# PaddlePaddle/PaddleNLP

Hardware: NVIDIA H100
Metric: tokens/sec Llama-3.2-3B seq4096 bf16 pretrain step (global, all GPUs) (higher is better)
Workload: dtype bf16

## Files before the change

paddlenlp_b200/csrc/common.cuh:

```cuda
#pragma once
#include <cuda.h>
#include <cuda_bf16.h>
#include <cuda_runtime.h>
#include <stdint.h>
#include <stdio.h>

namespace b200 {

typedef __nv_bfloat16 bf16;

__device__ __forceinline__ uint32_t smem_u32(const void* p) {
  return static_cast<uint32_t>(__cvta_generic_to_shared(p));
}
__device__ __forceinline__ void named_bar_sync(uint32_t id, uint32_t nthreads) {
  asm volatile("bar.sync %0, %1;" ::"r"(id), "r"(nthreads) : "memory");
}

__device__ __forceinline__ void pdl_wait() { asm volatile("griddepcontrol.wait;" ::: "memory"); }
__device__ __forceinline__ void pdl_launch_dependents() { asm volatile("griddepcontrol.launch_dependents;" ::: "memory"); }

__device__ __forceinline__ void mbar_init(uint64_t* bar, uint32_t count) {
  asm volatile("mbarrier.init.shared::cta.b64 [%0], %1;" ::"r"(smem_u32(bar)), "r"(count) : "memory");
}
__device__ __forceinline__ void fence_mbar_init() {
  asm volatile("fence.mbarrier_init.release.cluster;" ::: "memory");
}
__device__ __forceinline__ void fence_proxy_async_smem() {
  asm volatile("fence.proxy.async.shared::cta;" ::: "memory");
}
__device__ __forceinline__ void mbar_arrive_expect_tx(uint64_t* bar, uint32_t bytes) {
  asm volatile("mbarrier.arrive.expect_tx.shared::cta.b64 _, [%0], %1;" ::"r"(smem_u32(bar)), "r"(bytes)
               : "memory");
}
__device__ __forceinline__ void mbar_arrive(uint64_t* bar) {
  asm volatile("mbarrier.arrive.shared::cta.b64 _, [%0];" ::"r"(smem_u32(bar)) : "memory");
}
__device__ __forceinline__ bool mbar_try_wait(uint64_t* bar, uint32_t parity) {
  uint32_t ok;
  asm volatile(
      "{\n\t.reg .pred P;\n\t"
      "mbarrier.try_wait.parity.shared::cta.b64 P, [%1], %2;\n\t"
      "selp.u32 %0, 1, 0, P;\n\t}\n"
      : "=r"(ok)
      : "r"(smem_u32(bar)), "r"(parity)
      : "memory");
  return ok != 0;
}
__device__ __forceinline__ void mbar_wait(uint64_t* bar, uint32_t parity) {
  if (mbar_try_wait(bar, parity)) return;
  long long t0 = clock64();
  uint32_t spins = 0;
  while (!mbar_try_wait(bar, parity)) {
    if ((++spins & 0x3FFu) == 0 && (clock64() - t0) > 8000000000LL) {
      printf("[b200 watchdog] mbarrier wait timed out: block %d thread %d bar 0x%x parity %u\n", (int)blockIdx.x,
             (int)threadIdx.x, smem_u32(bar), parity);
      __trap();
    }
  }
}
__device__ __forceinline__ void mbar_wait_nocall(uint64_t* bar, uint32_t parity) {
  if (mbar_try_wait(bar, parity)) return;
  long long t0 = clock64();
  uint32_t spins = 0;
  while (!mbar_try_wait(bar, parity)) {
    if ((++spins & 0x3FFu) == 0 && (clock64() - t0) > 8000000000LL) __trap();
  }
}

__device__ __forceinline__ void tma_prefetch_desc(const CUtensorMap* tm) {
  asm volatile("prefetch.tensormap [%0];" ::"l"(reinterpret_cast<uint64_t>(tm)) : "memory");
}
__device__ __forceinline__ void tma_load_2d(const CUtensorMap* tm, uint64_t* bar, void* smem_dst, int c0, int c1) {
  asm volatile(
      "cp.async.bulk.tensor.2d.shared::cluster.global.mbarrier::complete_tx::bytes [%0], [%1, {%3, %4}], [%2];"
      ::"r"(smem_u32(smem_dst)), "l"(reinterpret_cast<uint64_t>(tm)), "r"(smem_u32(bar)), "r"(c0), "r"(c1)
      : "memory");
}
__device__ __forceinline__ void bulk_load(void* smem_dst, const void* src, uint32_t bytes, uint64_t* bar) {
  asm volatile("cp.async.bulk.shared::cluster.global.mbarrier::complete_tx::bytes [%0], [%1], %2, [%3];" ::"r"(smem_u32(smem_dst)),
               "l"(src), "r"(bytes), "r"(smem_u32(bar))
               : "memory");
}
__device__ __forceinline__ void tma_load_4d(const CUtensorMap* tm, uint64_t* bar, void* smem_dst, int c0, int c1,
                                            int c2, int c3) {
  asm volatile(
      "cp.async.bulk.tensor.4d.shared::cluster.global.mbarrier::complete_tx::bytes [%0], [%1, {%3, %4, %5, %6}], [%2];"
      ::"r"(smem_u32(smem_dst)), "l"(reinterpret_cast<uint64_t>(tm)), "r"(smem_u32(bar)), "r"(c0), "r"(c1), "r"(c2),
      "r"(c3)
      : "memory");
}
__device__ __forceinline__ void tma_reduce_add_4d(const CUtensorMap* tm, const void* smem_src, int c0, int c1, int c2,
                                                  int c3) {
  asm volatile("cp.reduce.async.bulk.tensor.4d.global.shared::cta.add.tile.bulk_group [%0, {%2, %3, %4, %5}], [%1];" ::"l"(
                   reinterpret_cast<uint64_t>(tm)),
               "r"(smem_u32(smem_src)), "r"(c0), "r"(c1), "r"(c2), "r"(c3)
               : "memory");
}
__device__ __forceinline__ void tma_reduce_add_2d(const CUtensorMap* tm, uint32_t smem_src, int c0, int c1) {
  asm volatile("cp.reduce.async.bulk.tensor.2d.global.shared::cta.add.tile.bulk_group [%0, {%2, %3}], [%1];" ::"l"(
                   reinterpret_cast<uint64_t>(tm)),
               "r"(smem_src), "r"(c0), "r"(c1)
               : "memory");
}
__device__ __forceinline__ void tma_store_2d(const CUtensorMap* tm, uint32_t smem_src, int c0, int c1) {
  asm volatile("cp.async.bulk.tensor.2d.global.shared::cta.bulk_group [%0, {%2, %3}], [%1];" ::"l"(reinterpret_cast<uint64_t>(tm)),
               "r"(smem_src), "r"(c0), "r"(c1)
               : "memory");
}
__device__ __forceinline__ void tma_prefetch_l2_2d(const CUtensorMap* tm, int c0, int c1) {
  asm volatile("cp.async.bulk.prefetch.tensor.2d.L2.global.tile [%0, {%1, %2}];" ::"l"(reinterpret_cast<uint64_t>(tm)), "r"(c0),
               "r"(c1)
               : "memory");
}
__device__ __forceinline__ void tma_store_commit() { asm volatile("cp.async.bulk.commit_group;" ::: "memory"); }
template <int N>
__device__ __forceinline__ void tma_store_wait_read() {
  asm volatile("cp.async.bulk.wait_group.read %0;" ::"n"(N) : "memory");
}
template <int N>
__device__ __forceinline__ void tma_store_wait() {
  asm volatile("cp.async.bulk.wait_group %0;" ::"n"(N) : "memory");
}

__device__ __forceinline__ uint64_t wgmma_desc_sw128(uint32_t saddr, uint32_t lbo_bytes, uint32_t sbo_bytes) {
  uint64_t d = 0;
  d |= static_cast<uint64_t>((saddr & 0x3FFFFu) >> 4);
  d |= static_cast<uint64_t>((lbo_bytes >> 4) & 0x3FFFu) << 16;
  d |= static_cast<uint64_t>((sbo_bytes >> 4) & 0x3FFFu) << 32;
  d |= static_cast<uint64_t>(1) << 62;
  return d;
}
__device__ __forceinline__ void wgmma_fence() { asm volatile("wgmma.fence.sync.aligned;" ::: "memory"); }
__device__ __forceinline__ void wgmma_commit() { asm volatile("wgmma.commit_group.sync.aligned;" ::: "memory"); }
template <int N>
__device__ __forceinline__ void wgmma_wait() { asm volatile("wgmma.wait_group.sync.aligned %0;" ::"n"(N) : "memory"); }
template <int R>
__device__ __forceinline__ void setmaxnreg_dec() { asm volatile("setmaxnreg.dec.sync.aligned.u32 %0;" ::"n"(R)); }
template <int R>
__device__ __forceinline__ void setmaxnreg_inc() { asm volatile("setmaxnreg.inc.sync.aligned.u32 %0;" ::"n"(R)); }

template <int TA, int TB>
__device__ __forceinline__ void wgmma_m64n256k16(float (&d)[128], uint64_t desc_a, uint64_t desc_b, uint32_t accumulate) {
  asm volatile(
      "{\n\t.reg .pred p;\n\tsetp.ne.b32 p, %130, 0;\n\t"
      "wgmma.mma_async.sync.aligned.m64n256k16.f32.bf16.bf16 "
      "{%0, %1, %2, %3, %4, %5, %6, %7, %8, %9, %10, %11, %12, %13, %14, %15, %16, %17, %18, %19, %20, %21, %22, %23, %24, %25, %26, %27, %28, %29, %30, %31, %32, %33, %34, %35, %36, %37, %38, %39, %40, %41, %42, %43, %44, %45, %46, %47, %48, %49, %50, %51, %52, %53, %54, %55, %56, %57, %58, %59, %60, %61, %62, %63, %64, %65, %66, %67, %68, %69, %70, %71, %72, %73, %74, %75, %76, %77, %78, %79, %80, %81, %82, %83, %84, %85, %86, %87, %88, %89, %90, %91, %92, %93, %94, %95, %96, %97, %98, %99, %100, %101, %102, %103, %104, %105, %106, %107, %108, %109, %110, %111, %112, %113, %114, %115, %116, %117, %118, %119, %120, %121, %122, %123, %124, %125, %126, %127}, %128, %129, p, 1, 1, %131, %132;\n\t}\n"
      : "+f"(d[0]), "+f"(d[1]), "+f"(d[2]), "+f"(d[3]), "+f"(d[4]), "+f"(d[5]), "+f"(d[6]), "+f"(d[7]), "+f"(d[8]), "+f"(d[9]), "+f"(d[10]), "+f"(d[11]), "+f"(d[12]), "+f"(d[13]), "+f"(d[14]), "+f"(d[15]), "+f"(d[16]), "+f"(d[17]), "+f"(d[18]), "+f"(d[19]), "+f"(d[20]), "+f"(d[21]), "+f"(d[22]), "+f"(d[23]), "+f"(d[24]), "+f"(d[25]), "+f"(d[26]), "+f"(d[27]), "+f"(d[28]), "+f"(d[29]), "+f"(d[30]), "+f"(d[31]), "+f"(d[32]), "+f"(d[33]), "+f"(d[34]), "+f"(d[35]), "+f"(d[36]), "+f"(d[37]), "+f"(d[38]), "+f"(d[39]), "+f"(d[40]), "+f"(d[41]), "+f"(d[42]), "+f"(d[43]), "+f"(d[44]), "+f"(d[45]), "+f"(d[46]), "+f"(d[47]), "+f"(d[48]), "+f"(d[49]), "+f"(d[50]), "+f"(d[51]), "+f"(d[52]), "+f"(d[53]), "+f"(d[54]), "+f"(d[55]), "+f"(d[56]), "+f"(d[57]), "+f"(d[58]), "+f"(d[59]), "+f"(d[60]), "+f"(d[61]), "+f"(d[62]), "+f"(d[63]), "+f"(d[64]), "+f"(d[65]), "+f"(d[66]), "+f"(d[67]), "+f"(d[68]), "+f"(d[69]), "+f"(d[70]), "+f"(d[71]), "+f"(d[72]), "+f"(d[73]), "+f"(d[74]), "+f"(d[75]), "+f"(d[76]), "+f"(d[77]), "+f"(d[78]), "+f"(d[79]), "+f"(d[80]), "+f"(d[81]), "+f"(d[82]), "+f"(d[83]), "+f"(d[84]), "+f"(d[85]), "+f"(d[86]), "+f"(d[87]), "+f"(d[88]), "+f"(d[89]), "+f"(d[90]), "+f"(d[91]), "+f"(d[92]), "+f"(d[93]), "+f"(d[94]), "+f"(d[95]), "+f"(d[96]), "+f"(d[97]), "+f"(d[98]), "+f"(d[99]), "+f"(d[100]), "+f"(d[101]), "+f"(d[102]), "+f"(d[103]), "+f"(d[104]), "+f"(d[105]), "+f"(d[106]), "+f"(d[107]), "+f"(d[108]), "+f"(d[109]), "+f"(d[110]), "+f"(d[111]), "+f"(d[112]), "+f"(d[113]), "+f"(d[114]), "+f"(d[115]), "+f"(d[116]), "+f"(d[117]), "+f"(d[118]), "+f"(d[119]), "+f"(d[120]), "+f"(d[121]), "+f"(d[122]), "+f"(d[123]), "+f"(d[124]), "+f"(d[125]), "+f"(d[126]), "+f"(d[127])
      : "l"(desc_a), "l"(desc_b), "r"(accumulate), "n"(TA), "n"(TB));
}
template <int TA, int TB>
__device__ __forceinline__ void wgmma_m64n64k16(float (&d)[32], uint64_t desc_a, uint64_t desc_b, uint32_t accumulate) {
  asm volatile(
      "{\n\t.reg .pred p;\n\tsetp.ne.b32 p, %34, 0;\n\t"
      "wgmma.mma_async.sync.aligned.m64n64k16.f32.bf16.bf16 "
      "{%0, %1, %2, %3, %4, %5, %6, %7, %8, %9, %10, %11, %12, %13, %14, %15, %16, %17, %18, %19, %20, %21, %22, %23, %24, %25, %26, %27, %28, %29, %30, %31}, %32, %33, p, 1, 1, %35, %36;\n\t}\n"
      : "+f"(d[0]), "+f"(d[1]), "+f"(d[2]), "+f"(d[3]), "+f"(d[4]), "+f"(d[5]), "+f"(d[6]), "+f"(d[7]), "+f"(d[8]), "+f"(d[9]), "+f"(d[10]), "+f"(d[11]), "+f"(d[12]), "+f"(d[13]), "+f"(d[14]), "+f"(d[15]), "+f"(d[16]), "+f"(d[17]), "+f"(d[18]), "+f"(d[19]), "+f"(d[20]), "+f"(d[21]), "+f"(d[22]), "+f"(d[23]), "+f"(d[24]), "+f"(d[25]), "+f"(d[26]), "+f"(d[27]), "+f"(d[28]), "+f"(d[29]), "+f"(d[30]), "+f"(d[31])
      : "l"(desc_a), "l"(desc_b), "r"(accumulate), "n"(TA), "n"(TB));
}
template <int TA, int TB>
__device__ __forceinline__ void wgmma_m64n128k16(float (&d)[64], uint64_t desc_a, uint64_t desc_b, uint32_t accumulate) {
  asm volatile(
      "{\n\t.reg .pred p;\n\tsetp.ne.b32 p, %66, 0;\n\t"
      "wgmma.mma_async.sync.aligned.m64n128k16.f32.bf16.bf16 "
      "{%0, %1, %2, %3, %4, %5, %6, %7, %8, %9, %10, %11, %12, %13, %14, %15, %16, %17, %18, %19, %20, %21, %22, %23, %24, %25, %26, %27, %28, %29, %30, %31, %32, %33, %34, %35, %36, %37, %38, %39, %40, %41, %42, %43, %44, %45, %46, %47, %48, %49, %50, %51, %52, %53, %54, %55, %56, %57, %58, %59, %60, %61, %62, %63}, %64, %65, p, 1, 1, %67, %68;\n\t}\n"
      : "+f"(d[0]), "+f"(d[1]), "+f"(d[2]), "+f"(d[3]), "+f"(d[4]), "+f"(d[5]), "+f"(d[6]), "+f"(d[7]), "+f"(d[8]), "+f"(d[9]), "+f"(d[10]), "+f"(d[11]), "+f"(d[12]), "+f"(d[13]), "+f"(d[14]), "+f"(d[15]), "+f"(d[16]), "+f"(d[17]), "+f"(d[18]), "+f"(d[19]), "+f"(d[20]), "+f"(d[21]), "+f"(d[22]), "+f"(d[23]), "+f"(d[24]), "+f"(d[25]), "+f"(d[26]), "+f"(d[27]), "+f"(d[28]), "+f"(d[29]), "+f"(d[30]), "+f"(d[31]), "+f"(d[32]), "+f"(d[33]), "+f"(d[34]), "+f"(d[35]), "+f"(d[36]), "+f"(d[37]), "+f"(d[38]), "+f"(d[39]), "+f"(d[40]), "+f"(d[41]), "+f"(d[42]), "+f"(d[43]), "+f"(d[44]), "+f"(d[45]), "+f"(d[46]), "+f"(d[47]), "+f"(d[48]), "+f"(d[49]), "+f"(d[50]), "+f"(d[51]), "+f"(d[52]), "+f"(d[53]), "+f"(d[54]), "+f"(d[55]), "+f"(d[56]), "+f"(d[57]), "+f"(d[58]), "+f"(d[59]), "+f"(d[60]), "+f"(d[61]), "+f"(d[62]), "+f"(d[63])
      : "l"(desc_a), "l"(desc_b), "r"(accumulate), "n"(TA), "n"(TB));
}
template <int TB>
// ... 152 lines not shown
```

paddlenlp_b200/csrc/fa_bwd.cu:

```cuda
#include <climits>

#include "../../include/b200nlp.h"
#include "common.cuh"
#include "host_util.h"

namespace b200 {
namespace fab {

constexpr int BKV = 64;
constexpr int NUM_THREADS = 256;

struct Params {
  const bf16 *q, *k, *v, *dout;
  int64_t ldq, ldk, ldv, lddo;
  int S, B, nh, kvh, Spad;
  float scale, scale_log2;
  const float* lse2;
  const float* delta;
  const int* mask_start;
  float* dq_acc;
  float* dk_acc;
  float* dv_acc;
};

// ... 74 lines not shown
          ldsm_x4(sV + swz<D>(kr, kc * 2 + ((lane >> 3) & 1)), bv);
          mma_bf16_16816(s[2 * np], a, b[0], b[1]);
          mma_bf16_16816(s[2 * np + 1], a, b[2], b[3]);
          mma_bf16_16816(dp[2 * np], ad, bv[0], bv[1]);
          mma_bf16_16816(dp[2 * np + 1], ad, bv[2], bv[3]);
        }
      }
#pragma unroll
      for (int h = 0; h < 2; ++h) {
        const int rl = rg * 16 + g + 8 * h, r = q0 + rl;
        const float lse2 = s_lse[rl], dl = s_delta[rl];
#pragma unroll
        for (int nt = 0; nt < NT; ++nt) {
          float pv[2], dsv[2];
#pragma unroll
          for (int e = 0; e < 2; ++e) {
            const int c = kv0 + cs * NT * 8 + nt * 8 + 2 * tq + e;
            bool dead = c > r;
            if constexpr (MASK) {
              if (!dead && c < p.S) dead = r >= __ldg(p.mask_start + tok0 + c);
            }
            pv[e] = dead ? 0.f : fast_exp2(fmaf(s[nt][2 * h + e], p.scale_log2, -lse2));
            dsv[e] = pv[e] * (dp[nt][2 * h + e] - dl) * p.scale;
          }
          const int cc = cs * NT + nt;
          asm volatile("st.shared.b32 [%0], %1;" ::"r"(sP + swz64(rl, cc) + tq * 4), "r"(pack_bf16x2(pv[0], pv[1])) : "memory");
          asm volatile("st.shared.b32 [%0], %1;" ::"r"(sdS + swz64(rl, cc) + tq * 4), "r"(pack_bf16x2(dsv[0], dsv[1])) : "memory");
        }
      }
    }
    __syncthreads();

#pragma unroll
    for (int qc = 0; qc < BQ / 16; ++qc) {
      uint32_t ap[4], as[4];
      const int pr = qc * 16 + (lane & 7) + ((lane >> 4) << 3), pc = kg * 2 + ((lane >> 3) & 1);
      ldsm_x4_t(sP + swz64(pr, pc), ap);
      ldsm_x4_t(sdS + swz64(pr, pc), as);
#pragma unroll
      for (int dp2 = 0; dp2 < D / 32; ++dp2) {
        const int br = qc * 16 + (lane & 7) + ((lane >> 3) & 1) * 8, bc = dh * (DCH / 2) + dp2 * 2 + (lane >> 4);
        uint32_t bo[4], bq[4];
        ldsm_x4_t(sdO + swz<D>(br, bc), bo);
        ldsm_x4_t(sQ + swz<D>(br, bc), bq);
        mma_bf16_16816(dv[2 * dp2], ap, bo[0], bo[1]);
        mma_bf16_16816(dv[2 * dp2 + 1], ap, bo[2], bo[3]);
        mma_bf16_16816(dk[2 * dp2], as, bq[0], bq[1]);
        mma_bf16_16816(dk[2 * dp2 + 1], as, bq[2], bq[3]);
      }
    }
    {
      const int qg = warp % QG, dsl = warp / QG;
      float dq[DTQ][4];
#pragma unroll
      for (int i = 0; i < DTQ; ++i) dq[i][0] = dq[i][1] = dq[i][2] = dq[i][3] = 0.f;
#pragma unroll
      for (int kc = 0; kc < BKV / 16; ++kc) {
        uint32_t a[4];
        ldsm_x4(sdS + swz64(qg * 16 + (lane & 15), kc * 2 + (lane >> 4)), a);
#pragma unroll
        for (int dp2 = 0; dp2 < DTQ / 2; ++dp2) {
          uint32_t b[4];
          ldsm_x4_t(sK + swz<D>(kc * 16 + (lane & 7) + ((lane >> 3) & 1) * 8, dsl * (DTQ) + dp2 * 2 + (lane >> 4)), b);
          mma_bf16_16816(dq[2 * dp2], a, b[0], b[1]);
          mma_bf16_16816(dq[2 * dp2 + 1], a, b[2], b[3]);
        }
      }
#pragma unroll
      for (int h = 0; h < 2; ++h) {
        const int r = q0 + qg * 16 + g + 8 * h;
        if (r >= p.S) continue;
        float* dst = p.dq_acc + ((tok0 + r) * p.nh + head) * D + dsl * DTQ * 8 + 2 * tq;
#pragma unroll
        for (int dt = 0; dt < DTQ; ++dt) {
          atomicAdd(dst + dt * 8, dq[dt][2 * h]);
          atomicAdd(dst + dt * 8 + 1, dq[dt][2 * h + 1]);
        }
      }
    }
    __syncthreads();
  }
#pragma unroll
  for (int h = 0; h < 2; ++h) {
    const int r = kv0 + kg * 16 + g + 8 * h;
    if (r >= p.S) continue;
    const size_t off = ((tok0 + r) * p.kvh + kv_head) * D + dh * (D / 2) + 2 * tq;
#pragma unroll
    for (int dt = 0; dt < D / 16; ++dt) {
      atomicAdd(p.dk_acc + off + dt * 8, dk[dt][2 * h]);
      atomicAdd(p.dk_acc + off + dt * 8 + 1, dk[dt][2 * h + 1]);
      atomicAdd(p.dv_acc + off + dt * 8, dv[dt][2 * h]);
      atomicAdd(p.dv_acc + off + dt * 8 + 1, dv[dt][2 * h + 1]);
    }
  }
}

template <int D>
__global__ void fa_bwd_delta_kernel(const bf16* __restrict__ o, const bf16* __restrict__ dout, const float* __restrict__ lse,
                                    float* __restrict__ lse2, float* __restrict__ delta, int B, int S, int Spad, int nh,
                                    int64_t ldo, int64_t lddo) {
  constexpr int LPR = D / 8, LPR_LOG2 = D == 128 ? 4 : 3;
  const int64_t row = (blockIdx.x * static_cast<int64_t>(blockDim.x) + threadIdx.x) >> LPR_LOG2;
  const int sub = threadIdx.x & (LPR - 1);
  const int64_t total = static_cast<int64_t>(B) * Spad * nh;
  float acc = 0.f;
  int b = 0, s = 0, h = 0;
  if (row < total) {
    h = static_cast<int>(row % nh);
    s = static_cast<int>((row / nh) % Spad);
    b = static_cast<int>(row / nh / Spad);
  }
  if (row < total && s < S) {
    const int64_t tok = static_cast<int64_t>(b) * S + s;
    const uint4 ov = ld_nc_v4(reinterpret_cast<const uint4*>(o + tok * ldo + h * D) + sub);
    const uint4 dv = ld_nc_v4(reinterpret_cast<const uint4*>(dout + tok * lddo + h * D) + sub);
    const uint32_t* oi = reinterpret_cast<const uint32_t*>(&ov);
    const uint32_t* di = reinterpret_cast<const uint32_t*>(&dv);
#pragma unroll
    for (int j = 0; j < 4; ++j) {
      const float2 a = unpack_bf16x2(oi[j]), d = unpack_bf16x2(di[j]);
      acc += a.x * d.x + a.y * d.y;
    }
  }
#pragma unroll
  for (int off = LPR / 2; off > 0; off >>= 1) acc += __shfl_xor_sync(0xffffffffu, acc, off);
  if (row < total && sub == 0) {
    const size_t bh = static_cast<size_t>(b) * nh + h;
    delta[bh * Spad + s] = acc;
    lse2[bh * Spad + s] = s < S ? lse[bh * S + s] * 1.4426950408889634f : INFINITY;
  }
}

__global__ void fa_bwd_dq_finish_kernel(const float* __restrict__ acc, bf16* __restrict__ dq, int64_t tokens, int width,
                                        int64_t lddq) {
  const int64_t nchunk_row = width >> 3;
  const int64_t total = tokens * nchunk_row;
  for (int64_t i = blockIdx.x * static_cast<int64_t>(blockDim.x) + threadIdx.x; i < total;
       i += static_cast<int64_t>(gridDim.x) * blockDim.x) {
    const int64_t t = i / nchunk_row, c = i % nchunk_row;
    const float4* src = reinterpret_cast<const float4*>(acc + t * width) + 2 * c;
    const float4 a = src[0], b = src[1];
    uint4 o;
    o.x = pack_bf16x2(a.x, a.y); o.y = pack_bf16x2(a.z, a.w);
    o.z = pack_bf16x2(b.x, b.y); o.w = pack_bf16x2(b.z, b.w);
    *(reinterpret_cast<uint4*>(dq + t * lddq) + c) = o;
  }
}

namespace wg {
constexpr int BKV = 128;
constexpr int BQ = 64;
constexpr int STAGES = 2;
constexpr int NUM_THREADS = 256;
constexpr int HK = BKV * 64 * 2;
constexpr int HQ = BQ * 64 * 2;

template <int D>
struct Layout {
  static constexpr int KV_BYTES = BKV * D * 2;
  static constexpr int QT_BYTES = BQ * D * 2;
  static constexpr int STAGE_BYTES = 2 * QT_BYTES + 2 * BQ * 4;
  static constexpr int STAGE_STRIDE = (STAGE_BYTES + 1023) / 1024 * 1024;
  static constexpr int DS_BYTES = BKV * BQ * 2;
  static constexpr int DQ_BYTES = BQ * 64 * 4;
  static constexpr int OFF_K = 0, OFF_V = KV_BYTES, OFF_RING = 2 * KV_BYTES;
  static constexpr int OFF_DS = OFF_RING + STAGES * STAGE_STRIDE;
  static constexpr int OFF_DQ = OFF_DS + 2 * DS_BYTES;
  static constexpr int OFF_BAR = OFF_DQ + 2 * DQ_BYTES;
  static constexpr int SMEM_BYTES = OFF_BAR + 64 + 1024;
  static_assert(SMEM_BYTES <= 227 * 1024, "fa_bwd_wgmma: shared memory");
  static_assert(64 * D * 4 <= STAGE_STRIDE && 64 * D * 4 <= 2 * DS_BYTES && 64 * D * 4 <= 2 * DQ_BYTES,
                "fa_bwd_wgmma: shared-memory layout");
};
static_assert(Layout<128>::STAGE_STRIDE == 33 * 1024, "fa_bwd_wgmma: head_dim 128 layout");

struct Params {
  int S, nh, kvh, Spad;
  float scale, scale_log2;
  const float* lse2;
  const float* delta;
  const int* mask_start;
};

template <int N>
__device__ __forceinline__ void reg_fence(float (&r)[N]) {
#pragma unroll
  for (int i = 0; i < N; ++i) asm volatile("" : "+f"(r[i])::"memory");
}

template <int NJ>
__device__ __forceinline__ void stage_f32(uint32_t base, const float (&acc)[4 * NJ], int wi, int lane) {
  const int g = lane >> 2, tq = lane & 3;
#pragma unroll
  for (int i = 0; i < 2; ++i) {
    const int row = wi * 16 + g + 8 * i;
#pragma unroll
    for (int j = 0; j < NJ; ++j) {
      const int chunk = (j & 3) * 2 + (tq >> 1);
      const uint32_t a = base + (j >> 2) * (64 * 128) + row * 128 + ((chunk ^ (row & 7)) << 4) + (tq & 1) * 8;
      asm volatile("st.shared.v2.f32 [%0], {%1, %2};" ::"r"(a), "f"(acc[4 * j + 2 * i]), "f"(acc[4 * j + 2 * i + 1]) : "memory");
    }
  }
}

template <int D, bool MASK>
__global__ void __launch_bounds__(NUM_THREADS, 1)
fa_bwd_wgmma_kernel(const __grid_constant__ CUtensorMap tmQ, const __grid_constant__ CUtensorMap tmK,
                    const __grid_constant__ CUtensorMap tmV, const __grid_constant__ CUtensorMap tmdO,
                    const __grid_constant__ CUtensorMap tmdQ, const __grid_constant__ CUtensorMap tmdK,
                    const __grid_constant__ CUtensorMap tmdV, const Params p) {
  using L = Layout<D>;
  constexpr int KV_BYTES = L::KV_BYTES, QT_BYTES = L::QT_BYTES, STAGE_BYTES = L::STAGE_BYTES, STAGE_STRIDE = L::STAGE_STRIDE;
  constexpr int DS_BYTES = L::DS_BYTES, DQ_BYTES = L::DQ_BYTES;
  constexpr int OFF_K = L::OFF_K, OFF_V = L::OFF_V, OFF_RING = L::OFF_RING, OFF_DS = L::OFF_DS, OFF_DQ = L::OFF_DQ, OFF_BAR = L::OFF_BAR;
  extern __shared__ uint8_t smem_raw[];
  uint8_t* smem = reinterpret_cast<uint8_t*>((reinterpret_cast<uintptr_t>(smem_raw) + 1023) & ~uintptr_t(1023));
  uint64_t* full_bar = reinterpret_cast<uint64_t*>(smem + OFF_BAR);
  uint64_t* empty_bar = full_bar + STAGES;
  uint64_t* kv_bar = empty_bar + STAGES;

  const int head = static_cast<int>(blockIdx.x) % p.nh, batch = static_cast<int>(blockIdx.x) / p.nh;
  const int kv_head = head / (p.nh / p.kvh);
  const int kv0 = static_cast<int>(blockIdx.y) * BKV;
  int q_lo = kv0 / BQ, q_hi = (p.S + BQ - 1) / BQ;
  if constexpr (MASK) {
    const int last = __ldg(p.mask_start + static_cast<size_t>(batch) * p.S + min(kv0 + BKV - 1, p.S - 1));
    q_hi = min(q_hi, (last + BQ - 1) / BQ);
  }
  if (threadIdx.x == 0) {
    tma_prefetch_desc(&tmQ); tma_prefetch_desc(&tmK); tma_prefetch_desc(&tmV); tma_prefetch_desc(&tmdO);
    tma_prefetch_desc(&tmdQ); tma_prefetch_desc(&tmdK); tma_prefetch_desc(&tmdV);
    for (int i = 0; i < STAGES; ++i) {
      mbar_init(&full_bar[i], 1);
      mbar_init(&empty_bar[i], 256);
    }
    mbar_init(kv_bar, 1);
    fence_mbar_init();
  }
  __syncthreads();

  const size_t stat0 = (static_cast<size_t>(batch) * p.nh + head) * p.Spad;
  auto load_q_tile = [&](int qt, int st) {
    uint8_t* sq = smem + OFF_RING + st * STAGE_STRIDE;
    mbar_arrive_expect_tx(&full_bar[st], STAGE_BYTES);
#pragma unroll
    for (int h = 0; h < D / 64; ++h) {
      tma_load_4d(&tmQ, &full_bar[st], sq + h * HQ, h * 64, head, qt * BQ, batch);
      tma_load_4d(&tmdO, &full_bar[st], sq + QT_BYTES + h * HQ, h * 64, head, qt * BQ, batch);
    }
    bulk_load(sq + 2 * QT_BYTES, p.lse2 + stat0 + qt * BQ, BQ * 4, &full_bar[st]);
    bulk_load(sq + 2 * QT_BYTES + BQ * 4, p.delta + stat0 + qt * BQ, BQ * 4, &full_bar[st]);
  };
  if (threadIdx.x == 0) {
    mbar_arrive_expect_tx(kv_bar, 2 * KV_BYTES);
#pragma unroll
    for (int h = 0; h < D / 64; ++h) {
      tma_load_4d(&tmK, kv_bar, smem + OFF_K + h * HK, h * 64, kv_head, kv0, batch);
      tma_load_4d(&tmV, kv_bar, smem + OFF_V + h * HK, h * 64, kv_head, kv0, batch);
    }
    for (int i = 0; i < STAGES && q_lo + i < q_hi; ++i) load_q_tile(q_lo + i, i);
  }

  const int cw = threadIdx.x >> 7;
  const int wi = (threadIdx.x >> 5) & 3, lane = threadIdx.x & 31, g = lane >> 2, tq = lane & 3;
  const bool leader = (threadIdx.x & 127) == 0;
  const uint32_t sbase = smem_u32(smem);
  const uint32_t sK = sbase + OFF_K, sV = sbase + OFF_V;
  const int kv_r = kv0 + cw * 64 + wi * 16 + g;
  int ms[2] = {INT_MAX, INT_MAX};
  if constexpr (MASK) {
#pragma unroll
    for (int i = 0; i < 2; ++i)
      if (kv_r + 8 * i < p.S) ms[i] = __ldg(p.mask_start + static_cast<size_t>(batch) * p.S + kv_r + 8 * i);
  }
  float dk[D / 2], dv[D / 2];
#pragma unroll
  for (int i = 0; i < D / 2; ++i) dk[i] = dv[i] = 0.f;
  mbar_wait_nocall(kv_bar, 0);

  for (int qt = q_lo, it = 0; qt < q_hi; ++qt, ++it) {
    const int st = it % STAGES, q0 = qt * BQ;
    const uint32_t sQ = sbase + OFF_RING + st * STAGE_STRIDE, sdO = sQ + QT_BYTES;
    const float* s_lse = reinterpret_cast<const float*>(smem + OFF_RING + st * STAGE_STRIDE + 2 * QT_BYTES);
    const float* s_delta = s_lse + BQ;
    if (threadIdx.x == 0 && it > 0 && qt - 1 + STAGES < q_hi) {
      const int ps = (it - 1) % STAGES;
      mbar_wait_nocall(&empty_bar[ps], ((it - 1) / STAGES) & 1);
      load_q_tile(qt - 1 + STAGES, ps);
    }
    mbar_wait_nocall(&full_bar[st], (it / STAGES) & 1);

    float s[32];
    wgmma_fence();
#pragma unroll
    for (int kk = 0; kk < D / 16; ++kk) {
      const uint32_t ko = (kk >> 2) * HK + cw * 64 * 128 + (kk & 3) * 32, qo = (kk >> 2) * HQ + (kk & 3) * 32;
      wgmma_m64n64k16<0, 0>(s, wgmma_desc_sw128(sK + ko, 16, 1024), wgmma_desc_sw128(sQ + qo, 16, 1024), kk > 0 ? 1u : 0u);
    }
    wgmma_commit();
    wgmma_wait<0>();
    reg_fence(s);
#pragma unroll
    for (int j = 0; j < 8; ++j) {
#pragma unroll
      for (int e = 0; e < 2; ++e) {
        const int c = 8 * j + 2 * tq + e, r = q0 + c;
        const float l2 = s_lse[c];
#pragma unroll
        for (int i = 0; i < 2; ++i) {
          bool dead = kv_r + 8 * i > r;
          if constexpr (MASK) dead = dead || r >= ms[i];
          float& x = s[4 * j + 2 * i + e];
          x = dead ? 0.f : fast_exp2(fmaf(x, p.scale_log2, -l2));
        }
      }
    }
    float dp[32];
    wgmma_fence();
#pragma unroll
    for (int kk = 0; kk < D / 16; ++kk) {
      const uint32_t ko = (kk >> 2) * HK + cw * 64 * 128 + (kk & 3) * 32, qo = (kk >> 2) * HQ + (kk & 3) * 32;
      wgmma_m64n64k16<0, 0>(dp, wgmma_desc_sw128(sV + ko, 16, 1024), wgmma_desc_sw128(sdO + qo, 16, 1024), kk > 0 ? 1u : 0u);
    }
    wgmma_commit();
    wgmma_wait<0>();
    reg_fence(dp);
#pragma unroll
    for (int j = 0; j < 8; ++j) {
#pragma unroll
      for (int e = 0; e < 2; ++e) {
        const float dl = s_delta[8 * j + 2 * tq + e];
#pragma unroll
        for (int i = 0; i < 2; ++i) {
          float& x = dp[4 * j + 2 * i + e];
          x = s[4 * j + 2 * i + e] * (x - dl) * p.scale;
        }
      }
    }
    uint32_t pa[16], da[16];
#pragma unroll
    for (int t = 0; t < 16; ++t) {
      pa[t] = pack_bf16x2(s[2 * t], s[2 * t + 1]);
      da[t] = pack_bf16x2(dp[2 * t], dp[2 * t + 1]);
    }
    wgmma_fence();
    if constexpr (D == 128) {
#pragma unroll
      for (int k = 0; k < 4; ++k) wgmma_m64n128k16_rs<1>(dv, pa + 4 * k, wgmma_desc_sw128(sdO + k * 2048, HQ, 1024), 1u);
#pragma unroll
      for (int k = 0; k < 4; ++k) wgmma_m64n128k16_rs<1>(dk, da + 4 * k, wgmma_desc_sw128(sQ + k * 2048, HQ, 1024), 1u);
    } else {
#pragma unroll
      for (int k = 0; k < 4; ++k) wgmma_m64n64k16_rs<1>(dv, pa + 4 * k, wgmma_desc_sw128(sdO + k * 2048, HQ, 1024), 1u);
#pragma unroll
      for (int k = 0; k < 4; ++k) wgmma_m64n64k16_rs<1>(dk, da + 4 * k, wgmma_desc_sw128(sQ + k * 2048, HQ, 1024), 1u);
    }
    wgmma_commit();
    const uint32_t sdS = sbase + OFF_DS + (it & 1) * DS_BYTES;
#pragma unroll
    for (int i = 0; i < 2; ++i) {
      const int row = cw * 64 + wi * 16 + g + 8 * i;
#pragma unroll
      for (int j = 0; j < 8; ++j)
        asm volatile("st.shared.b32 [%0], %1;" ::"r"(sdS + row * 128 + ((j ^ (row & 7)) << 4) + tq * 4), "r"(da[2 * j + i]) : "memory");
    }
    fence_proxy_async_smem();
    float dq[32];
    if constexpr (D == 128) {
      named_bar_sync(1, 256);
#pragma unroll
      for (int kk = 0; kk < 8; ++kk)
        wgmma_m64n64k16<1, 1>(dq, wgmma_desc_sw128(sdS + kk * 2048, DS_BYTES, 1024),
                              wgmma_desc_sw128(sK + cw * HK + kk * 2048, HK, 1024), kk > 0 ? 1u : 0u);
    } else {
      named_bar_sync(2 + cw, 128);
#pragma unroll
      for (int kk = 0; kk < 4; ++kk)
        wgmma_m64n64k16<1, 1>(dq, wgmma_desc_sw128(sdS + cw * 64 * 128 + kk * 2048, DS_BYTES, 1024),
                              wgmma_desc_sw128(sK + cw * 64 * 128 + kk * 2048, HK, 1024), kk > 0 ? 1u : 0u);
    }
    wgmma_commit();
    wgmma_wait<0>();
    reg_fence(dq);
    reg_fence(dk);
    reg_fence(dv);
    mbar_arrive(&empty_bar[st]);
    uint8_t* sdq = smem + OFF_DQ + cw * DQ_BYTES;
    if (leader) tma_store_wait_read<0>();
    named_bar_sync(2 + cw, 128);
    stage_f32<8>(smem_u32(sdq), dq, wi, lane);
    fence_proxy_async_smem();
    named_bar_sync(2 + cw, 128);
    if (leader) {
      const int d0 = D == 128 ? cw * 64 : 0;
      tma_reduce_add_4d(&tmdQ, sdq, d0, head, q0, batch);
      tma_reduce_add_4d(&tmdQ, sdq + DQ_BYTES / 2, d0 + 32, head, q0, batch);
      tma_store_commit();
    }
  }

  if (leader) tma_store_wait_read<0>();
  named_bar_sync(1, 256);
  uint8_t* sdk = smem + OFF_RING + cw * STAGE_STRIDE;
  uint8_t* sdv = smem + (cw == 0 ? OFF_DS : OFF_DQ);
  stage_f32<D / 8>(smem_u32(sdk), dk, wi, lane);
  stage_f32<D / 8>(smem_u32(sdv), dv, wi, lane);
  fence_proxy_async_smem();
  named_bar_sync(2 + cw, 128);
  if (leader) {
#pragma unroll
    for (int b = 0; b < D / 32; ++b) {
      tma_reduce_add_4d(&tmdK, sdk + b * (64 * 128), b * 32, kv_head, kv0 + cw * 64, batch);
      tma_reduce_add_4d(&tmdV, sdv + b * (64 * 128), b * 32, kv_head, kv0 + cw * 64, batch);
    }
    tma_store_commit();
    tma_store_wait<0>();
  }
}

static int make_f32_map(CUtensorMap* tm, float* base, int64_t B, int64_t S, int64_t heads, int64_t D) {
  const uint64_t dims[4] = {static_cast<uint64_t>(D), static_cast<uint64_t>(heads), static_cast<uint64_t>(S), static_cast<uint64_t>(B)};
  const uint64_t row = static_cast<uint64_t>(D) * 4;
  const uint64_t strides[3] = {row, static_cast<uint64_t>(heads) * row, static_cast<uint64_t>(S * heads) * row};
  const uint32_t box[4] = {32, 1, 64, 1};
  return encode_tmap_f32(tm, base, 4, dims, strides, box);
}

template <int D, bool MASK>
static int launch(const CUtensorMap (&tm)[7], const Params& p, int B, cudaStream_t stream) {
  constexpr int SMEM_BYTES = Layout<D>::SMEM_BYTES;
  auto kern = fa_bwd_wgmma_kernel<D, MASK>;
  static bool attr_set = false;
  if (!attr_set) {
    cudaError_t e = cudaFuncSetAttribute(kern, cudaFuncAttributeMaxDynamicSharedMemorySize, SMEM_BYTES);
    if (e != cudaSuccess) {
      set_last_error("fa_bwd_wgmma smem attr: %s", cudaGetErrorString(e));
      return static_cast<int>(e);
    }
    attr_set = true;
  }
  const dim3 grid(static_cast<unsigned>(p.nh * B), static_cast<unsigned>((p.S + BKV - 1) / BKV));
  kern<<<grid, NUM_THREADS, SMEM_BYTES, stream>>>(tm[0], tm[1], tm[2], tm[3], tm[4], tm[5], tm[6], p);
  return check_launch("fa_bwd_wgmma");
}
}

template <int D, int BQ, bool MASK>
static int launch(const Params& p, cudaStream_t stream) {
  constexpr int SMEM = 2 * BKV * D * 2 + 2 * BQ * D * 2 + 2 * BQ * 128 + 2 * BQ * 4;
  static bool attr_set = false;
  if (!attr_set) {
    cudaError_t e = cudaFuncSetAttribute(fa_bwd_kernel<D, BQ, MASK>, cudaFuncAttributeMaxDynamicSharedMemorySize, SMEM);
    if (e != cudaSuccess) {
      set_last_error("fa_bwd smem attr: %s", cudaGetErrorString(e));
      return static_cast<int>(e);
    }
    attr_set = true;
  }
  dim3 grid(static_cast<unsigned>((p.S + BKV - 1) / BKV), static_cast<unsigned>(p.nh), static_cast<unsigned>(p.B));
  fa_bwd_kernel<D, BQ, MASK><<<grid, NUM_THREADS, SMEM, stream>>>(p);
  return check_launch("fa_bwd");
}

}
}

extern "C" int64_t b200_fa_bwd_workspace_bytes(int64_t B, int64_t S, int64_t num_heads, int64_t head_dim) {
  const int64_t Spad = (S + 63) / 64 * 64;
  return 3 * B * Spad * num_heads * head_dim * 4 + B * num_heads * Spad * 8;
}

extern "C" int b200_fa_bwd(const void* q, const void* k, const void* v, const void* o, const void* dout, const float* lse,
                           void* dq, void* dk, void* dv, void* workspace, int64_t B, int64_t S, int64_t num_heads,
                           int64_t num_kv_heads, int64_t head_dim, int64_t ldq, int64_t ldk, int64_t ldv, int64_t ldo,
                           int64_t lddo, int64_t lddq, int64_t lddk, int64_t lddv, float softmax_scale,
                           cudaStream_t stream) {
  return b200_fa_bwd_flashmask(q, k, v, o, dout, lse, nullptr, dq, dk, dv, workspace, B, S, num_heads, num_kv_heads, head_dim,
                               ldq, ldk, ldv, ldo, lddo, lddq, lddk, lddv, softmax_scale, stream);
}

extern "C" int b200_fa_bwd_flashmask(const void* q, const void* k, const void* v, const void* o, const void* dout,
                                     const float* lse, const int32_t* mask_start_rows, void* dq, void* dk, void* dv,
                                     void* workspace, int64_t B, int64_t S, int64_t num_heads, int64_t num_kv_heads,
                                     int64_t head_dim, int64_t ldq, int64_t ldk, int64_t ldv, int64_t ldo, int64_t lddo,
                                     int64_t lddq, int64_t lddk, int64_t lddv, float softmax_scale, cudaStream_t stream) {
  using namespace b200;
  using namespace b200::fab;
  B200_CHECK_ARG(q && k && v && o && dout && lse && dq && dk && dv && workspace, "fa_bwd: null pointer");
  B200_CHECK_ARG(head_dim == 64 || head_dim == 128, "fa_bwd: head_dim must be 64 or 128 (got %lld)", (long long)head_dim);
  B200_CHECK_ARG(B > 0 && S > 0 && num_heads > 0 && num_kv_heads > 0 && num_heads % num_kv_heads == 0, "fa_bwd: bad shape");
  B200_CHECK_ARG(ldq % 8 == 0 && ldk % 8 == 0 && ldv % 8 == 0 && ldo % 8 == 0 && lddo % 8 == 0 && lddq % 8 == 0 &&
                     lddk % 8 == 0 && lddv % 8 == 0,
                 "fa_bwd: token strides must be multiples of 8");
  {
    const void* ptrs[8] = {q, k, v, o, dout, dq, dk, dv};
    const char* names[8] = {"q", "k", "v", "o", "dout", "dq", "dk", "dv"};
    for (int i = 0; i < 8; ++i)
      B200_CHECK_ARG((reinterpret_cast<uintptr_t>(ptrs[i]) & 15) == 0, "fa_bwd: %s must be 16-byte aligned (got %p)", names[i], ptrs[i]);
  }
  const int64_t Spad = (S + 63) / 64 * 64;
  float* dq_acc = static_cast<float*>(workspace);
  float* dk_acc = dq_acc + B * S * num_heads * head_dim;
  float* dv_acc = dk_acc + B * S * num_kv_heads * head_dim;
  float* lse2 = dq_acc + 3 * B * S * num_heads * head_dim;
  float* delta = lse2 + B * num_heads * Spad;
  cudaError_t e = cudaMemsetAsync(dq_acc, 0, static_cast<size_t>(B) * S * (num_heads + 2 * num_kv_heads) * head_dim * 4, stream);
  if (e != cudaSuccess) {
    set_last_error("fa_bwd memset: %s", cudaGetErrorString(e));
    return static_cast<int>(e);
  }
  {
    const int64_t rows = B * Spad * num_heads;
    const int64_t threads = rows * (head_dim / 8);
    const unsigned blocks = static_cast<unsigned>((threads + 255) / 256);
    const bf16 *op = static_cast<const bf16*>(o), *dop = static_cast<const bf16*>(dout);
    if (head_dim == 64)
      fa_bwd_delta_kernel<64><<<blocks, 256, 0, stream>>>(op, dop, lse, lse2, delta, (int)B, (int)S, (int)Spad, (int)num_heads, ldo, lddo);
    else
      fa_bwd_delta_kernel<128><<<blocks, 256, 0, stream>>>(op, dop, lse, lse2, delta, (int)B, (int)S, (int)Spad, (int)num_heads, ldo, lddo);
    int rc = check_launch("fa_bwd(delta)");
    if (rc) return rc;
  }
  int rc;
  if (fa_bwd_impl() == 1) {
    Params p;
    p.q = static_cast<const bf16*>(q); p.k = static_cast<const bf16*>(k); p.v = static_cast<const bf16*>(v);
    p.dout = static_cast<const bf16*>(dout);
    p.ldq = ldq; p.ldk = ldk; p.ldv = ldv; p.lddo = lddo;
    p.S = (int)S; p.B = (int)B; p.nh = (int)num_heads; p.kvh = (int)num_kv_heads; p.Spad = (int)Spad;
    p.scale = softmax_scale;
    p.scale_log2 = softmax_scale * 1.4426950408889634f;
    p.lse2 = lse2; p.delta = delta;
    p.mask_start = mask_start_rows;
    p.dq_acc = dq_acc; p.dk_acc = dk_acc; p.dv_acc = dv_acc;
    if (head_dim == 64)
      rc = mask_start_rows ? launch<64, 64, true>(p, stream) : launch<64, 64, false>(p, stream);
    else
      rc = mask_start_rows ? launch<128, 64, true>(p, stream) : launch<128, 64, false>(p, stream);
  } else {
    CUtensorMap tm[7];
    if ((rc = make_bf16_map(&tm[0], q, B, S, num_heads, head_dim, ldq, wg::BQ)) != 0) return rc;
    if ((rc = make_bf16_map(&tm[1], k, B, S, num_kv_heads, head_dim, ldk, wg::BKV)) != 0) return rc;
    if ((rc = make_bf16_map(&tm[2], v, B, S, num_kv_heads, head_dim, ldv, wg::BKV)) != 0) return rc;
    if ((rc = make_bf16_map(&tm[3], dout, B, S, num_heads, head_dim, lddo, wg::BQ)) != 0) return rc;
    if ((rc = wg::make_f32_map(&tm[4], dq_acc, B, S, num_heads, head_dim)) != 0) return rc;
    if ((rc = wg::make_f32_map(&tm[5], dk_acc, B, S, num_kv_heads, head_dim)) != 0) return rc;
    if ((rc = wg::make_f32_map(&tm[6], dv_acc, B, S, num_kv_heads, head_dim)) != 0) return rc;
    wg::Params p;
    p.S = (int)S; p.nh = (int)num_heads; p.kvh = (int)num_kv_heads; p.Spad = (int)Spad;
    p.scale = softmax_scale;
    p.scale_log2 = softmax_scale * 1.4426950408889634f;
    p.lse2 = lse2; p.delta = delta;
    p.mask_start = mask_start_rows;
    if (head_dim == 64)
      rc = mask_start_rows ? wg::launch<64, true>(tm, p, (int)B, stream) : wg::launch<64, false>(tm, p, (int)B, stream);
    else
      rc = mask_start_rows ? wg::launch<128, true>(tm, p, (int)B, stream) : wg::launch<128, false>(tm, p, (int)B, stream);
  }
  if (rc) return rc;
  {
    const int64_t tokens = B * S;
    const int width = static_cast<int>(num_heads * head_dim);
    const int64_t total = tokens * (width / 8);
    int64_t blocks = (total + 255) / 256;
    const int64_t cap = static_cast<int64_t>(sm_count()) * 16;
    if (blocks > cap) blocks = cap;
    fa_bwd_dq_finish_kernel<<<static_cast<unsigned>(blocks), 256, 0, stream>>>(dq_acc, static_cast<bf16*>(dq), tokens,
                                                                              width, lddq);
    if ((rc = check_launch("fa_bwd(dq finish)")) != 0) return rc;
    const int kvw = static_cast<int>(num_kv_heads * head_dim);
    int64_t kblocks = (tokens * (kvw / 8) + 255) / 256;
    if (kblocks > cap) kblocks = cap;
    fa_bwd_dq_finish_kernel<<<static_cast<unsigned>(kblocks), 256, 0, stream>>>(dk_acc, static_cast<bf16*>(dk), tokens, kvw,
                                                                               lddk);
    if ((rc = check_launch("fa_bwd(dk finish)")) != 0) return rc;
    fa_bwd_dq_finish_kernel<<<static_cast<unsigned>(kblocks), 256, 0, stream>>>(dv_acc, static_cast<bf16*>(dv), tokens, kvw,
                                                                               lddv);
    rc = check_launch("fa_bwd(dv finish)");
  }
  return rc;
}
```

Baseline: 24450.

## Software-pipeline dQ GEMM across Q tiles and regroup FA backward grid

Restructures the WGMMA flash-attention backward loop so the dQ GEMM for the previous Q tile is issued alongside the dK/dV GEMMs of the current tile. Split named barriers (arrive/sync pairs on double-buffered dS) replace the full-CTA sync. The S and dP GEMMs are now issued back to back and awaited separately, and the causal mask is skipped on fully unmasked tiles. The grid becomes 1D with batch-head grouping for better L2 reuse of K/V across CTAs. This adds barrier complexity and register pressure, since dq is live alongside dk/dv.

```diff
diff --git a/paddlenlp_b200/csrc/common.cuh b/paddlenlp_b200/csrc/common.cuh
--- a/paddlenlp_b200/csrc/common.cuh
+++ b/paddlenlp_b200/csrc/common.cuh
@@ -14,6 +14,9 @@
 }
 __device__ __forceinline__ void named_bar_sync(uint32_t id, uint32_t nthreads) {
   asm volatile("bar.sync %0, %1;" ::"r"(id), "r"(nthreads) : "memory");
+}
+__device__ __forceinline__ void named_bar_arrive(uint32_t id, uint32_t nthreads) {
+  asm volatile("bar.arrive %0, %1;" ::"r"(id), "r"(nthreads) : "memory");
 }
 
 __device__ __forceinline__ void pdl_wait() { asm volatile("griddepcontrol.wait;" ::: "memory"); }
diff --git a/paddlenlp_b200/csrc/fa_bwd.cu b/paddlenlp_b200/csrc/fa_bwd.cu
--- a/paddlenlp_b200/csrc/fa_bwd.cu
+++ b/paddlenlp_b200/csrc/fa_bwd.cu
@@ -250,6 +250,7 @@
 constexpr int BQ = 64;
 constexpr int STAGES = 2;
 constexpr int NUM_THREADS = 256;
+constexpr int BH_GROUP = 32;
 constexpr int HK = BKV * 64 * 2;
 constexpr int HQ = BQ * 64 * 2;
 
@@ -285,6 +286,11 @@
 #pragma unroll
   for (int i = 0; i < N; ++i) asm volatile("" : "+f"(r[i])::"memory");
 }
+template <int N>
+__device__ __forceinline__ void reg_fence(uint32_t (&r)[N]) {
+#pragma unroll
+  for (int i = 0; i < N; ++i) asm volatile("" : "+r"(r[i])::"memory");
+}
 
 template <int NJ>
 __device__ __forceinline__ void stage_f32(uint32_t base, const float (&acc)[4 * NJ], int wi, int lane) {
@@ -317,9 +323,16 @@
   uint64_t* empty_bar = full_bar + STAGES;
   uint64_t* kv_bar = empty_bar + STAGES;
 
-  const int head = static_cast<int>(blockIdx.x) % p.nh, batch = static_cast<int>(blockIdx.x) / p.nh;
+  int bh, kv_tile;
+  {
+    const int lin = static_cast<int>(blockIdx.x), n_kv = (p.S + BKV - 1) / BKV, n_bh = static_cast<int>(gridDim.x) / n_kv;
+    const int g0 = lin / (BH_GROUP * n_kv) * BH_GROUP, gn = min(BH_GROUP, n_bh - g0), r = lin - g0 * n_kv;
+    kv_tile = r / gn;
+    bh = g0 + r % gn;
+  }
+  const int head = bh % p.nh, batch = bh / p.nh;
   const int kv_head = head / (p.nh / p.kvh);
-  const int kv0 = static_cast<int>(blockIdx.y) * BKV;
+  const int kv0 = kv_tile * BKV;
   int q_lo = kv0 / BQ, q_hi = (p.S + BQ - 1) / BQ;
   if constexpr (MASK) {
     const int last = __ldg(p.mask_start + static_cast<size_t>(batch) * p.S + min(kv0 + BKV - 1, p.S - 1));
@@ -376,113 +389,26 @@
   for (int i = 0; i < D / 2; ++i) dk[i] = dv[i] = 0.f;
   mbar_wait_nocall(kv_bar, 0);
 
-  for (int qt = q_lo, it = 0; qt < q_hi; ++qt, ++it) {
-    const int st = it % STAGES, q0 = qt * BQ;
-    const uint32_t sQ = sbase + OFF_RING + st * STAGE_STRIDE, sdO = sQ + QT_BYTES;
-    const float* s_lse = reinterpret_cast<const float*>(smem + OFF_RING + st * STAGE_STRIDE + 2 * QT_BYTES);
-    const float* s_delta = s_lse + BQ;
-    if (threadIdx.x == 0 && it > 0 && qt - 1 + STAGES < q_hi) {
-      const int ps = (it - 1) % STAGES;
-      mbar_wait_nocall(&empty_bar[ps], ((it - 1) / STAGES) & 1);
-      load_q_tile(qt - 1 + STAGES, ps);
-    }
-    mbar_wait_nocall(&full_bar[st], (it / STAGES) & 1);
-
-    float s[32];
-    wgmma_fence();
-#pragma unroll
-    for (int kk = 0; kk < D / 16; ++kk) {
-      const uint32_t ko = (kk >> 2) * HK + cw * 64 * 128 + (kk & 3) * 32, qo = (kk >> 2) * HQ + (kk & 3) * 32;
-      wgmma_m64n64k16<0, 0>(s, wgmma_desc_sw128(sK + ko, 16, 1024), wgmma_desc_sw128(sQ + qo, 16, 1024), kk > 0 ? 1u : 0u);
-    }
-    wgmma_commit();
-    wgmma_wait<0>();
-    reg_fence(s);
-#pragma unroll
-    for (int j = 0; j < 8; ++j) {
-#pragma unroll
-      for (int e = 0; e < 2; ++e) {
-        const int c = 8 * j + 2 * tq + e, r = q0 + c;
-        const float l2 = s_lse[c];
-#pragma unroll
-        for (int i = 0; i < 2; ++i) {
-          bool dead = kv_r + 8 * i > r;
-          if constexpr (MASK) dead = dead || r >= ms[i];
-          float& x = s[4 * j + 2 * i + e];
-          x = dead ? 0.f : fast_exp2(fmaf(x, p.scale_log2, -l2));
-        }
-      }
-    }
-    float dp[32];
-    wgmma_fence();
-#pragma unroll
-    for (int kk = 0; kk < D / 16; ++kk) {
-      const uint32_t ko = (kk >> 2) * HK + cw * 64 * 128 + (kk & 3) * 32, qo = (kk >> 2) * HQ + (kk & 3) * 32;
-      wgmma_m64n64k16<0, 0>(dp, wgmma_desc_sw128(sV + ko, 16, 1024), wgmma_desc_sw128(sdO + qo, 16, 1024), kk > 0 ? 1u : 0u);
-    }
-    wgmma_commit();
-    wgmma_wait<0>();
-    reg_fence(dp);
-#pragma unroll
-    for (int j = 0; j < 8; ++j) {
-#pragma unroll
-      for (int e = 0; e < 2; ++e) {
-        const float dl = s_delta[8 * j + 2 * tq + e];
-#pragma unroll
-        for (int i = 0; i < 2; ++i) {
-          float& x = dp[4 * j + 2 * i + e];
-          x = s[4 * j + 2 * i + e] * (x - dl) * p.scale;
-        }
-      }
-    }
-    uint32_t pa[16], da[16];
-#pragma unroll
-    for (int t = 0; t < 16; ++t) {
-      pa[t] = pack_bf16x2(s[2 * t], s[2 * t + 1]);
-      da[t] = pack_bf16x2(dp[2 * t], dp[2 * t + 1]);
-    }
-    wgmma_fence();
+  auto issue_dq = [&](float (&dq)[32], int n) {
+    const uint32_t sdS = sbase + OFF_DS + (n & 1) * DS_BYTES;
     if constexpr (D == 128) {
-#pragma unroll
-      for (int k = 0; k < 4; ++k) wgmma_m64n128k16_rs<1>(dv, pa + 4 * k, wgmma_desc_sw128(sdO + k * 2048, HQ, 1024), 1u);
-#pragma unroll
-      for (int k = 0; k < 4; ++k) wgmma_m64n128k16_rs<1>(dk, da + 4 * k, wgmma_desc_sw128(sQ + k * 2048, HQ, 1024), 1u);
-    } else {
-#pragma unroll
-      for (int k = 0; k < 4; ++k) wgmma_m64n64k16_rs<1>(dv, pa + 4 * k, wgmma_desc_sw128(sdO + k * 2048, HQ, 1024), 1u);
-#pragma unroll
-      for (int k = 0; k < 4; ++k) wgmma_m64n64k16_rs<1>(dk, da + 4 * k, wgmma_desc_sw128(sQ + k * 2048, HQ, 1024), 1u);
-    }
-    wgmma_commit();
-    const uint32_t sdS = sbase + OFF_DS + (it & 1) * DS_BYTES;
-#pragma unroll
-    for (int i = 0; i < 2; ++i) {
-      const int row = cw * 64 + wi * 16 + g + 8 * i;
-#pragma unroll
-      for (int j = 0; j < 8; ++j)
-        asm volatile("st.shared.b32 [%0], %1;" ::"r"(sdS + row * 128 + ((j ^ (row & 7)) << 4) + tq * 4), "r"(da[2 * j + i]) : "memory");
-    }
-    fence_proxy_async_smem();
-    float dq[32];
-    if constexpr (D == 128) {
-      named_bar_sync(1, 256);
 #pragma unroll
       for (int kk = 0; kk < 8; ++kk)
         wgmma_m64n64k16<1, 1>(dq, wgmma_desc_sw128(sdS + kk * 2048, DS_BYTES, 1024),
                               wgmma_desc_sw128(sK + cw * HK + kk * 2048, HK, 1024), kk > 0 ? 1u : 0u);
     } else {
-      named_bar_sync(2 + cw, 128);
 #pragma unroll
       for (int kk = 0; kk < 4; ++kk)
         wgmma_m64n64k16<1, 1>(dq, wgmma_desc_sw128(sdS + cw * 64 * 128 + kk * 2048, DS_BYTES, 1024),
                               wgmma_desc_sw128(sK + cw * 64 * 128 + kk * 2048, HK, 1024), kk > 0 ? 1u : 0u);
     }
     wgmma_commit();
-    wgmma_wait<0>();
-    reg_fence(dq);
-    reg_fence(dk);
-    reg_fence(dv);
-    mbar_arrive(&empty_bar[st]);
+  };
+  auto wait_ds = [&](int n) {
+    if constexpr (D == 128) named_bar_sync(4 + 2 * (n & 1) + (cw ^ 1), 256);
+    else named_bar_sync(2 + cw, 128);
+  };
+  auto reduce_dq = [&](const float (&dq)[32], int n) {
     uint8_t* sdq = smem + OFF_DQ + cw * DQ_BYTES;
     if (leader) tma_store_wait_read<0>();
     named_bar_sync(2 + cw, 128);
@@ -491,10 +417,143 @@
     named_bar_sync(2 + cw, 128);
     if (leader) {
       const int d0 = D == 128 ? cw * 64 : 0;
-      tma_reduce_add_4d(&tmdQ, sdq, d0, head, q0, batch);
-      tma_reduce_add_4d(&tmdQ, sdq + DQ_BYTES / 2, d0 + 32, head, q0, batch);
+      tma_reduce_add_4d(&tmdQ, sdq, d0, head, (q_lo + n) * BQ, batch);
+      tma_reduce_add_4d(&tmdQ, sdq + DQ_BYTES / 2, d0 + 32, head, (q_lo + n) * BQ, batch);
       tma_store_commit();
     }
+  };
+
+  const int n_tiles = q_hi - q_lo;
+  for (int it = 0; it < n_tiles; ++it) {
+    const int qt = q_lo + it, st = it % STAGES, q0 = qt * BQ;
+    const uint32_t sQ = sbase + OFF_RING + st * STAGE_STRIDE, sdO = sQ + QT_BYTES;
+    const float* s_lse = reinterpret_cast<const float*>(smem + OFF_RING + st * STAGE_STRIDE + 2 * QT_BYTES);
+    const float* s_delta = s_lse + BQ;
+    if (threadIdx.x == 0 && it > 0 && qt - 1 + STAGES < q_hi) {
+      const int ps = (it - 1) % STAGES;
+      mbar_wait_nocall(&empty_bar[ps], ((it - 1) / STAGES) & 1);
+      load_q_tile(qt - 1 + STAGES, ps);
+    }
+    mbar_wait_nocall(&full_bar[st], (it / STAGES) & 1);
+
+    float s[32], dp[32];
+    wgmma_fence();
+#pragma unroll
+    for (int kk = 0; kk < D / 16; ++kk) {
+      const uint32_t ko = (kk >> 2) * HK + cw * 64 * 128 + (kk & 3) * 32, qo = (kk >> 2) * HQ + (kk & 3) * 32;
+      wgmma_m64n64k16<0, 0>(s, wgmma_desc_sw128(sK + ko, 16, 1024), wgmma_desc_sw128(sQ + qo, 16, 1024), kk > 0 ? 1u : 0u);
+    }
+    wgmma_commit();
+#pragma unroll
+    for (int kk = 0; kk < D / 16; ++kk) {
+      const uint32_t ko = (kk >> 2) * HK + cw * 64 * 128 + (kk & 3) * 32, qo = (kk >> 2) * HQ + (kk & 3) * 32;
+      wgmma_m64n64k16<0, 0>(dp, wgmma_desc_sw128(sV + ko, 16, 1024), wgmma_desc_sw128(sdO + qo, 16, 1024), kk > 0 ? 1u : 0u);
+    }
+    wgmma_commit();
+    wgmma_wait<1>();
+    reg_fence(s);
+    if (MASK || q0 < kv0 + BKV) {
+#pragma unroll
+      for (int j = 0; j < 8; ++j) {
+#pragma unroll
+        for (int e = 0; e < 2; ++e) {
+          const int c = 8 * j + 2 * tq + e, r = q0 + c;
+          const float l2 = s_lse[c];
+#pragma unroll
+          for (int i = 0; i < 2; ++i) {
+            bool dead = kv_r + 8 * i > r;
+            if constexpr (MASK) dead = dead || r >= ms[i];
+            float& x = s[4 * j + 2 * i + e];
+            x = dead ? 0.f : fast_exp2(fmaf(x, p.scale_log2, -l2));
+          }
+        }
+      }
+    } else {
+#pragma unroll
+      for (int j = 0; j < 8; ++j) {
+#pragma unroll
+        for (int e = 0; e < 2; ++e) {
+          const float l2 = s_lse[8 * j + 2 * tq + e];
+#pragma unroll
+          for (int i = 0; i < 2; ++i) {
+            float& x = s[4 * j + 2 * i + e];
+            x = fast_exp2(fmaf(x, p.scale_log2, -l2));
+          }
+        }
+      }
+    }
+    wgmma_wait<0>();
+    reg_fence(dp);
+#pragma unroll
+    for (int j = 0; j < 8; ++j) {
+#pragma unroll
+      for (int e = 0; e < 2; ++e) {
+        const float dl = s_delta[8 * j + 2 * tq + e];
+#pragma unroll
+        for (int i = 0; i < 2; ++i) {
+          float& x = dp[4 * j + 2 * i + e];
+          x = s[4 * j + 2 * i + e] * (x - dl) * p.scale;
+        }
+      }
+    }
+    uint32_t pa[16], da[16];
+#pragma unroll
+    for (int t = 0; t < 16; ++t) {
+      pa[t] = pack_bf16x2(s[2 * t], s[2 * t + 1]);
+      da[t] = pack_bf16x2(dp[2 * t], dp[2 * t + 1]);
+    }
+    if (it > 0) wait_ds(it - 1);
+    const uint32_t sdS = sbase + OFF_DS + (it & 1) * DS_BYTES;
+#pragma unroll
+    for (int i = 0; i < 2; ++i) {
+      const int row = cw * 64 + wi * 16 + g + 8 * i;
+#pragma unroll
+      for (int j = 0; j < 8; ++j)
+        asm volatile("st.shared.b32 [%0], %1;" ::"r"(sdS + row * 128 + ((j ^ (row & 7)) << 4) + tq * 4), "r"(da[2 * j + i]) : "memory");
+    }
+    fence_proxy_async_smem();
+    auto issue_dkdv = [&]() {
+      if constexpr (D == 128) {
+#pragma unroll
+        for (int k = 0; k < 4; ++k) wgmma_m64n128k16_rs<1>(dv, pa + 4 * k, wgmma_desc_sw128(sdO + k * 2048, HQ, 1024), 1u);
+#pragma unroll
+        for (int k = 0; k < 4; ++k) wgmma_m64n128k16_rs<1>(dk, da + 4 * k, wgmma_desc_sw128(sQ + k * 2048, HQ, 1024), 1u);
+      } else {
+#pragma unroll
+        for (int k = 0; k < 4; ++k) wgmma_m64n64k16_rs<1>(dv, pa + 4 * k, wgmma_desc_sw128(sdO + k * 2048, HQ, 1024), 1u);
+#pragma unroll
+        for (int k = 0; k < 4; ++k) wgmma_m64n64k16_rs<1>(dk, da + 4 * k, wgmma_desc_sw128(sQ + k * 2048, HQ, 1024), 1u);
+      }
+      wgmma_commit();
+    };
+    wgmma_fence();
+    if (it > 0) {
+      float dq[32];
+      issue_dq(dq, it - 1);
+      issue_dkdv();
+      wgmma_wait<1>();
+      reg_fence(dq);
+      if constexpr (D == 128) named_bar_arrive(4 + 2 * (it & 1) + cw, 256);
+      reduce_dq(dq, it - 1);
+    } else {
+      issue_dkdv();
+      if constexpr (D == 128) named_bar_arrive(4 + 2 * (it & 1) + cw, 256);
+    }
+    wgmma_wait<0>();
+    reg_fence(dk);
+    reg_fence(dv);
+    reg_fence(pa);
+    reg_fence(da);
+    mbar_arrive(&empty_bar[st]);
+  }
+  if (n_tiles > 0) {
+    wait_ds(n_tiles - 1);
+    float dq[32];
+    wgmma_fence();
+    issue_dq(dq, n_tiles - 1);
+    wgmma_wait<0>();
+    reg_fence(dq);
+    reduce_dq(dq, n_tiles - 1);
   }
 
   if (leader) tma_store_wait_read<0>();
@@ -537,7 +596,7 @@
     }
     attr_set = true;
   }
-  const dim3 grid(static_cast<unsigned>(p.nh * B), static_cast<unsigned>((p.S + BKV - 1) / BKV));
+  const dim3 grid(static_cast<unsigned>(p.nh * B * ((p.S + BKV - 1) / BKV)));
   kern<<<grid, NUM_THREADS, SMEM_BYTES, stream>>>(tm[0], tm[1], tm[2], tm[3], tm[4], tm[5], tm[6], p);
   return check_launch("fa_bwd_wgmma");
 }
```

Result: faster. 24740, median of 6 (+1.2%).
